# starlingonearth/MASt3R-SLAM-Quality-dualTSDF

Measured on AMD Instinct MI355X. Metric: SLAM frames/sec (infer+match+TSDF+GN) @512x384, higher is better.
Workload: dtype bf16

## Files before the change

include/mslam_hip.h:

```cpp
#ifndef MSLAM_HIP_H
#define MSLAM_HIP_H

#include <stddef.h>
#include <stdint.h>

#ifdef __cplusplus
extern "C" {
#endif

#define MSLAM_OK 0
#define MSLAM_EINVAL (-1)
#define MSLAM_EHIP (-2)
#define MSLAM_ENOMEM (-3)
#define MSLAM_ENODEV (-4)

const char* mslam_last_error(void);
int mslam_abi_version(void);
int mslam_device_check(void);


int mslam_iter_proj(const float* rays_img_with_grad, const float* pts_3d_norm,
                    const float* p_init, float* p_new, uint8_t* converged, int b, int h, int w,
                    int n, int max_iter, float lambda_init, float cost_thresh, void* stream);

int mslam_refine_matches(const uint16_t* D11, const uint16_t* D21, const int64_t* p1,
                         int64_t* p1_new, int b, int h, int w, int n, int fdim, int radius,
                         int dilation_max, void* stream);

int mslam_prep_iter_proj(const float* X11, const float* X21, const int64_t* idx_init,
                         float* rays_img_with_grad, float* pts_3d_norm, float* p_init, int b, int h,
                         int w, void* stream);

int mslam_match_occlusion(const float* X11, const float* X21, const float* p, int64_t* p1,
                          uint8_t* valid, int b, int h, int w, float dist_thresh, void* stream);

int mslam_pixel_to_lin(const int64_t* p1, int64_t* idx, int b, int n, int w, void* stream);

size_t mslam_gn_workspace_bytes(int num_poses, int num_edges, int num_points, int local_edges);

int mslam_gauss_newton_rays(float* Twc, const float* Xs, const float* Cs, const int64_t* ii,
                            const int64_t* jj, const int64_t* idx_ii2jj, const uint8_t* valid_match,
                            const float* Q, int num_poses, int num_points, int num_edges,
                            float sigma_ray, float sigma_dist, float C_thresh, float Q_thresh,
                            int max_iter, float delta_thresh, float* dx, void* workspace,
                            size_t workspace_bytes, void* stream);

int mslam_gauss_newton_calib(float* Twc, const float* Xs, const float* Cs, const float* K,
                             const int64_t* ii, const int64_t* jj, const int64_t* idx_ii2jj,
                             const uint8_t* valid_match, const float* Q, int num_poses, int num_points,
                             int num_edges, int height, int width, int pixel_border, float z_eps,
                             float sigma_pixel, float sigma_depth, float C_thresh, float Q_thresh,
                             int max_iter, float delta_thresh, float* dx, void* workspace,
                             size_t workspace_bytes, void* stream);

int mslam_gauss_newton_points(float* Twc, const float* Xs, const float* Cs, const int64_t* ii,
                              const int64_t* jj, const int64_t* idx_ii2jj, const uint8_t* valid_match,
                              const float* Q, int num_poses, int num_points, int num_edges,
                              float sigma_point, float C_thresh, float Q_thresh, int max_iter,
                              float delta_thresh, float* dx, void* workspace, size_t workspace_bytes,
// ... 265 lines not shown
                            uint8_t* out_count, void* stream);

#define MSLAM_IMAGE_METRICS_TILE_H 16
#define MSLAM_IMAGE_METRICS_TILE_W 32
size_t mslam_image_metrics_workspace_bytes(int n, int h, int w, int c);
int mslam_image_metrics(const float* a, const float* b, const uint8_t* mask, int n, int h, int w, int c,
                        const double* window, double* sums, int64_t* counts, float* ssim_map, void* workspace,
                        void* stream);

int mslam_mast3r_create(void** handle_out, const int* cfg9_host, void* const* weight_ptrs_host,
                        const long long* weight_numels_host, int n_weights, void* stream);
int mslam_mast3r_destroy(void* handle);
size_t mslam_mast3r_workspace_bytes(void* handle, int batch, int H, int W);

int mslam_mast3r_encode(void* handle, const float* img, int batch, int H, int W, float* feat_out,
                        void* workspace, size_t workspace_bytes, void* stream);

int mslam_mast3r_decode(void* handle, const float* feat1, const float* feat2, int batch, int H, int W,
                        float* X1, float* C1, float* D1, float* Q1, float* X2, float* C2, float* D2,
                        float* Q2, float* dec_last1, float* dec_last2, void* workspace,
                        size_t workspace_bytes, void* stream);

size_t mslam_track_workspace_bytes(int n_points);
int mslam_track_pose(int use_calib, float* T_rel, const float* Xf, const float* Xk, const int64_t* idx_f2k,
                     const float* Qk, const uint8_t* valid, int n_points, const float* K, int width,
                     int height, float sigma_a, float sigma_b, float huber, int pixel_border, float z_eps,
                     int first_iter, int max_iters, float rel_error, float delta_norm, void* status_out, void* workspace,
                     size_t workspace_bytes, void* stream);

size_t mslam_track_prepare_workspace_bytes(int n_points);
int mslam_track_prepare(const int64_t* idx_f2k, const uint8_t* valid_match, const float* Qff, const float* Qkf,
                        const float* Cf_sum, float inv_nf, const float* Ck_sum, float inv_nk, float C_conf, float Q_conf,
                        int n_points, const float* T_WCk, const float* T_WCf, float* Qk, float* Ck_avg,
                        uint8_t* valid_opt, uint8_t* valid_kf, float* T_rel, void* workspace, size_t workspace_bytes,
                        void* stream);
int mslam_track_verdict(const void* prepare_workspace, const void* status, int n_points, float* verdict6, void* stream);
int mslam_track_fuse(const float* T_WCk, const float* T_rel, const float* Xkf, const float* Ckf, const float* X_canon,
                     const float* C, int n_points, float* T_WCf, float* X_new, float* C_new, void* stream);

int mslam_gemm_bf16(const void* A, const void* W, const float* bias, const void* residual_f32, void* out,
                    int M, int N, int K, int act, int out_is_bf16, void* stream);
int mslam_gemm_tile_override(int M, int N, int K, int cfg);
int mslam_gemm_profile_begin(int M, int N, int K, int max_samples);
int mslam_gemm_profile_end(double* avg_us, double* min_us, int* samples);
int mslam_conv2d_nhwc_bf16(const void* in, const void* W, const float* bias, const void* residual_bf16,
                           void* out_bf16, int B, int H, int Wd, int Cin, int Cout, int ks, int stride,
// ... 64 lines not shown
```

mast3r-slam-quality-dualtsdf_amd/csrc/matching.hip:

```cpp
#include "common.h"

namespace mslam {

struct Bilin {
  float w11, w12, w21, w22;
  const float *r11, *r12, *r21, *r22;
};

__device__ __forceinline__ Bilin bilin_setup(const float* __restrict__ img, int w, float u, float v) {
  Bilin s;
  const int u11 = (int)floorf(u);
  const int v11 = (int)floorf(v);
  const float du = u - (float)u11;
  const float dv = v - (float)v11;
  const double dud = (double)du, dvd = (double)dv;
  const double omu = 1.0 - dud, omv = 1.0 - dvd;
  s.w11 = du * dv;
  s.w12 = (float)(omu * dvd);
  s.w21 = (float)(dud * omv);
  s.w22 = (float)(omu * omv);
  const float* base = img + ((size_t)v11 * w + u11) * 9;
  s.r22 = base;
  s.r21 = base + 9;
  s.r12 = base + (size_t)w * 9;
// ... 86 lines not shown
  converged[o] = conv;
}

typedef _Float16 h16;
typedef _Float16 h16x8 __attribute__((ext_vector_type(8)));

template <int FDIM>
__device__ __forceinline__ h16 half_dot_seq(const h16* __restrict__ a_regs, const h16* __restrict__ d11) {
  h16 score = (h16)0.0f;
  static_assert(FDIM % 8 == 0, "FDIM must be a multiple of 8");
#pragma unroll
  for (int c = 0; c < FDIM / 8; c++) {
    const h16x8 d = *reinterpret_cast<const h16x8*>(d11 + c * 8);
#pragma unroll
    for (int k = 0; k < 8; k++) {
      const h16 prod = a_regs[c * 8 + k] * d[k];
      score = score + prod;
    }
  }
  return score;
}

template <int FDIM>
__global__ __launch_bounds__(256) void refine_matches_kernel(
    const h16* __restrict__ D11, const h16* __restrict__ D21, const int64_t* __restrict__ p1,
    int64_t* __restrict__ p1_new, int h, int w, int n, int fdim_rt, int radius, int dilation_max) {
  const unsigned tile = xcd_remap(blockIdx.x, gridDim.x);
  const int i = tile * 256 + threadIdx.x;
  const int bi = blockIdx.y;
  if (i >= n) return;
  const int fdim = FDIM > 0 ? FDIM : fdim_rt;
  const h16* img = D11 + (size_t)bi * h * w * fdim;
  const size_t o = (size_t)bi * n + i;
  const h16* d21 = D21 + o * fdim;

  h16 a[FDIM > 0 ? FDIM : 1];
  if constexpr (FDIM > 0) {
#pragma unroll
    for (int c = 0; c < FDIM / 8; c++) {
      const h16x8 t = *reinterpret_cast<const h16x8*>(d21 + c * 8);
#pragma unroll
      for (int k = 0; k < 8; k++) a[c * 8 + k] = t[k];
    }
  }

  const longlong2 pp = *reinterpret_cast<const longlong2*>(p1 + o * 2);
  long long u0 = pp.x, v0 = pp.y;
  long long u_new = u0, v_new = v0;
  float max_score = 6.103515625e-05f;

  for (int d = dilation_max; d > 0; d--) {
    const int rd = radius * d;
    const int diam = 2 * rd + 1;
    for (int ii = 0; ii < diam; ii += d) {
      const long long u = u0 - rd + ii;
      const int ui = (int)u;
      if (ui < 0 || ui >= w) continue;
      for (int jj = 0; jj < diam; jj += d) {
        const long long v = v0 - rd + jj;
        const int vi = (int)v;
        if (vi < 0 || vi >= h) continue;
        const h16* d11 = img + ((unsigned)vi * (unsigned)w + (unsigned)ui) * (unsigned)fdim;
        h16 score;
        if constexpr (FDIM > 0) {
          score = half_dot_seq<FDIM>(a, d11);
        } else {
          score = (h16)0.0f;
          for (int k = 0; k < fdim; k++) {
            const h16 prod = d21[k] * d11[k];
            score = score + prod;
          }
        }
        const float sf = (float)score;
        if (sf > max_score) {
          max_score = sf;
          u_new = u;
          v_new = v;
        }
      }
    }
    u0 = u_new;
    v0 = v_new;
  }
  longlong2 out;
  out.x = u_new;
  out.y = v_new;
  *reinterpret_cast<longlong2*>(p1_new + o * 2) = out;
}

__device__ __forceinline__ int reflect_idx(int i, int n) {
  if (i < 0) return -i;
  if (i >= n) return 2 * n - 2 - i;
  return i;
}

__device__ __forceinline__ void normalize3(float x, float y, float z, float& ox, float& oy, float& oz) {
  const float nrm = fmaxf(sqrtf(fmaf(z, z, fmaf(y, y, x * x))), 1e-12f);
  ox = x / nrm;
  oy = y / nrm;
  oz = z / nrm;
}

constexpr int kPrepTile = 16;

__global__ __launch_bounds__(256) void prep_iter_proj_kernel(
    const float* __restrict__ X11, const float* __restrict__ X21, const int64_t* __restrict__ idx_init,
// ... 35 lines not shown
    gx = fmaf(-k3, a20, gx);
    gx = fmaf(k3, a22, gx);
    float gy = -k3 * a00;
    gy = fmaf(-k10, a01, gy);
    gy = fmaf(-k3, a02, gy);
    gy = fmaf(k3, a20, gy);
    gy = fmaf(k10, a21, gy);
    gy = fmaf(k3, a22, gy);
    out[c] = a11;
    out[3 + c] = gx;
    out[6 + c] = gy;
  }
  const float* q = X21 + o * 3;
  float a, b, c;
  normalize3(q[0], q[1], q[2], a, b, c);
  pts_out[o * 3 + 0] = a;
  pts_out[o * 3 + 1] = b;
  pts_out[o * 3 + 2] = c;
  const long long lin = idx_init ? idx_init[o] : (long long)pix;
  p_init[o * 2 + 0] = (float)(lin % w);
  p_init[o * 2 + 1] = (float)(lin / w);
}

__global__ __launch_bounds__(256) void match_occlusion_kernel(
    const float* __restrict__ X11, const float* __restrict__ X21, const float* __restrict__ p,
    int64_t* __restrict__ p1, uint8_t* __restrict__ valid, int h, int w, float dist_thresh) {
  const int n = h * w;
  const int i = blockIdx.x * 256 + threadIdx.x;
  const int bi = blockIdx.y;
  if (i >= n) return;
  const size_t o = (size_t)bi * n + i;
  const float2 pp = *reinterpret_cast<const float2*>(p + o * 2);
  const long long u = (long long)pp.x, v = (long long)pp.y;
  const float* a = X11 + ((size_t)bi * n + (size_t)v * w + (size_t)u) * 3;
  const float* q = X21 + o * 3;
  const float d0 = a[0] - q[0], d1 = a[1] - q[1], d2 = a[2] - q[2];
  const float dist = sqrtf(fmaf(d2, d2, fmaf(d1, d1, d0 * d0)));
  longlong2 out;
  out.x = u;
  out.y = v;
  *reinterpret_cast<longlong2*>(p1 + o * 2) = out;
  valid[o] = (valid[o] != 0) && (dist < dist_thresh);
}

__global__ __launch_bounds__(256) void pixel_to_lin_kernel(const int64_t* __restrict__ p1,
                                                           int64_t* __restrict__ idx, size_t total, int w) {
  const size_t i = (size_t)blockIdx.x * 256 + threadIdx.x;
  if (i >= total) return;
  const longlong2 pp = *reinterpret_cast<const longlong2*>(p1 + i * 2);
  idx[i] = pp.x + (long long)w * pp.y;
}

}

using namespace mslam;

extern "C" int mslam_iter_proj(const float* rays_img_with_grad, const float* pts_3d_norm,
                               const float* p_init, float* p_new, uint8_t* converged, int b, int h,
                               int w, int n, int max_iter, float lambda_init, float cost_thresh,
                               void* stream) {
  MSLAM_REQUIRE(b >= 0 && n >= 0 && max_iter >= 0, "iter_proj: negative size");
  if (b == 0 || n == 0) return MSLAM_OK;
  MSLAM_REQUIRE(rays_img_with_grad && pts_3d_norm && p_init && p_new && converged,
                "iter_proj: null pointer");
  MSLAM_REQUIRE(h >= 3 && w >= 3, "iter_proj: ray image must be at least 3x3 (got %dx%d)", h, w);
// ... 37 lines not shown
  MSLAM_REQUIRE(X11 && X21 && rays_img_with_grad && pts_3d_norm && p_init, "prep_iter_proj: null pointer");
  MSLAM_REQUIRE(h >= 2 && w >= 2, "prep_iter_proj: reflect padding needs h,w >= 2");
  MSLAM_REQUIRE(b <= 65535, "prep_iter_proj: batch %d exceeds grid limit", b);
  dim3 grid((w + kPrepTile - 1) / kPrepTile, (h + kPrepTile - 1) / kPrepTile, b);
  hipLaunchKernelGGL(prep_iter_proj_kernel, grid, dim3(256), 0, (hipStream_t)stream, X11, X21, idx_init,
                     rays_img_with_grad, pts_3d_norm, p_init, h, w);
  MSLAM_LAUNCH_CHECK("prep_iter_proj");
  return MSLAM_OK;
}

extern "C" int mslam_match_occlusion(const float* X11, const float* X21, const float* p, int64_t* p1,
                                     uint8_t* valid, int b, int h, int w, float dist_thresh,
                                     void* stream) {
  MSLAM_REQUIRE(b >= 0 && h >= 0 && w >= 0, "match_occlusion: negative size");
  if (b == 0 || h == 0 || w == 0) return MSLAM_OK;
  MSLAM_REQUIRE(X11 && X21 && p && p1 && valid, "match_occlusion: null pointer");
  dim3 grid((h * w + 255) / 256, b);
  hipLaunchKernelGGL(match_occlusion_kernel, grid, dim3(256), 0, (hipStream_t)stream, X11, X21, p, p1,
                     valid, h, w, dist_thresh);
  MSLAM_LAUNCH_CHECK("match_occlusion");
  return MSLAM_OK;
}

extern "C" int mslam_pixel_to_lin(const int64_t* p1, int64_t* idx, int b, int n, int w, void* stream) {
  MSLAM_REQUIRE(b >= 0 && n >= 0, "pixel_to_lin: negative size");
  const size_t total = (size_t)b * n;
  if (total == 0) return MSLAM_OK;
  MSLAM_REQUIRE(p1 && idx, "pixel_to_lin: null pointer");
  hipLaunchKernelGGL(pixel_to_lin_kernel, dim3((unsigned)((total + 255) / 256)), dim3(256), 0,
                     (hipStream_t)stream, p1, idx, total, w);
  MSLAM_LAUNCH_CHECK("pixel_to_lin");
  return MSLAM_OK;
}
```

mast3r-slam-quality-dualtsdf_amd/csrc/tracker.hip:

```cpp
#include "common.h"
#include "sim3.h"

namespace mslam {

constexpr int kTAcc = 36;

struct TrackState {
  int done;
  int iters;
  int chol_fail;
  float old_cost;
  float last_cost;
  float last_delta_norm;
  float pad0, pad1;
};

struct TrackParams {
  float inv_sigma_a, inv_sigma_b;
  float huber_k;
  const float* K;
  float border_lo, border_hi_u, border_hi_v, z_eps;
  int width;
};

__device__ __forceinline__ float huber_k(float r, float k) {
  const float a = fabsf(r);
  return a < k ? 1.0f : k / a;
}

template <unsigned NZ>
__device__ __forceinline__ void taccum_row(float (&acc)[kTAcc], const float (&x)[7], float w, float err) {
  const float we = w * err;
  int l = 0;
#pragma unroll
  for (int n = 0; n < 7; n++) {
    const float wx = w * x[n];
#pragma unroll
    for (int m = 0; m <= n; m++) {
      if (((NZ >> n) & 1u) && ((NZ >> m) & 1u)) acc[l] = fmaf(wx, x[m], acc[l]);
      l++;
    }
    if ((NZ >> n) & 1u) acc[28 + n] = fmaf(we, x[n], acc[28 + n]);
  }
  acc[35] = fmaf(we, err, acc[35]);
}

template <int CALIB>
__global__ __launch_bounds__(256) void track_accum_kernel(const TrackState* __restrict__ st,
                                                          const float* __restrict__ T,
                                                          const float* __restrict__ Xf, const float* __restrict__ Xk,
                                                          const int64_t* __restrict__ idx, const float* __restrict__ Qk,
                                                          const uint8_t* __restrict__ valid, int n, TrackParams P,
                                                          float* __restrict__ partial) {
  if (st->done) return;
  const Sim3f Tr = sim3_load(T);
  float R[9];
  quat_to_mat(Tr.q, R);
  float acc[kTAcc];
#pragma unroll
  for (int l = 0; l < kTAcc; l++) acc[l] = 0.0f;
  for (int k = blockIdx.x * 256 + threadIdx.x; k < n; k += gridDim.x * 256) {
    const long long j = idx[k];
    const float xf0 = Xf[j * 3], xf1 = Xf[j * 3 + 1], xf2 = Xf[j * 3 + 2];
    const float xk0 = Xk[(size_t)k * 3], xk1 = Xk[(size_t)k * 3 + 1], xk2 = Xk[(size_t)k * 3 + 2];
    const float p0 = Tr.s * (R[0] * xf0 + R[1] * xf1 + R[2] * xf2) + Tr.t[0];
    const float p1 = Tr.s * (R[3] * xf0 + R[4] * xf1 + R[5] * xf2) + Tr.t[1];
    const float p2 = Tr.s * (R[6] * xf0 + R[7] * xf1 + R[8] * xf2) + Tr.t[2];
    const float vq = valid[k] ? sqrtf(Qk[k]) : 0.0f;
    if constexpr (CALIB == 0) {
      const float nk = sqrtf(xk0 * xk0 + xk1 * xk1 + xk2 * xk2), nk_inv = 1.0f / nk;
      const float n2 = p0 * p0 + p1 * p1 + p2 * p2;
      const float np = sqrtf(n2), np_inv = 1.0f / np;
      const float r0 = p0 * np_inv, r1 = p1 * np_inv, r2 = p2 * np_inv;
      const float e0 = r0 - xk0 * nk_inv, e1 = r1 - xk1 * nk_inv, e2 = r2 - xk2 * nk_inv, e3 = np - nk;
      const float sa = P.inv_sigma_a * vq, sb = P.inv_sigma_b * vq;
      const float w0 = huber_k(sa * e0, P.huber_k) * sa * sa, w1 = huber_k(sa * e1, P.huber_k) * sa * sa;
      const float w2 = huber_k(sa * e2, P.huber_k) * sa * sa, w3 = huber_k(sb * e3, P.huber_k) * sb * sb;
      const float n3 = np_inv / n2;
// ... 21 lines not shown
      const float xz = p0 * zinv, yz = p1 * zinv;
      if (gate > 0.0f) {
        { const float x[7] = {Pfx * zinv, 0.0f, -Pfx * xz * zinv, -Pfx * xz * yz, Pfx * (1.0f + xz * xz), -Pfx * yz, 0.0f};
          taccum_row<0b0111101>(acc, x, w0, e0); }
        { const float x[7] = {0.0f, Pfy * zinv, -Pfy * yz * zinv, -Pfy * (1.0f + yz * yz), Pfy * xz * yz, Pfy * xz, 0.0f};
          taccum_row<0b0111110>(acc, x, w1, e1); }
        { const float x[7] = {0.0f, 0.0f, zinv, yz, -xz, 0.0f, 1.0f}; taccum_row<0b1011100>(acc, x, w2, e2); }
      }
    }
  }
  __shared__ float red[4][kTAcc];
  const int lane = threadIdx.x & 63, wid = threadIdx.x >> 6;
#pragma unroll
  for (int l = 0; l < kTAcc; l++) {
    const float s = wave_sum(acc[l]);
    if (lane == 0) red[wid][l] = s;
  }
  __syncthreads();
  if (threadIdx.x < kTAcc)
    partial[(size_t)blockIdx.x * kTAcc + threadIdx.x] =
        (red[0][threadIdx.x] + red[1][threadIdx.x]) + (red[2][threadIdx.x] + red[3][threadIdx.x]);
}

__global__ __launch_bounds__(64) void track_solve_kernel(TrackState* __restrict__ st, const float* __restrict__ partial,
                                                         int nblk, float* __restrict__ T, float rel_thresh,
                                                         float delta_thresh) {
  if (st->done) return;
  __shared__ double s[kTAcc];
  const int t = threadIdx.x;
  if (t < kTAcc) {
    double a = 0.0;
    for (int k = 0; k < nblk; k++) a += (double)partial[(size_t)k * kTAcc + t];
    s[t] = a;
  }
  __syncthreads();
  if (t != 0) return;
  double H[7][7], g[7];
  int l = 0;
  for (int n = 0; n < 7; n++)
    for (int m = 0; m <= n; m++) { H[n][m] = s[l]; H[m][n] = s[l]; l++; }
  for (int n = 0; n < 7; n++) g[n] = -s[28 + n];
  const float cost = (float)(0.5 * s[35]);
  double L[7][7];
  bool fail = false;
  for (int j = 0; j < 7 && !fail; j++) {
    double d = H[j][j];
    for (int k = 0; k < j; k++) d -= L[j][k] * L[j][k];
    if (!(d > 0.0)) { fail = true; break; }
    L[j][j] = sqrt(d);
    for (int i = j + 1; i < 7; i++) {
      double v = H[i][j];
      for (int k = 0; k < j; k++) v -= L[i][k] * L[j][k];
      L[i][j] = v / L[j][j];
    }
  }
  st->iters += 1;
  st->last_cost = cost;
  if (fail) { st->chol_fail = 1; st->done = 1; return; }
  double y[7], x[7];
  for (int i = 0; i < 7; i++) { double v = g[i]; for (int k = 0; k < i; k++) v -= L[i][k] * y[k]; y[i] = v / L[i][i]; }
  for (int i = 6; i >= 0; i--) { double v = y[i]; for (int k = i + 1; k < 7; k++) v -= L[k][i] * x[k]; x[i] = v / L[i][i]; }
  float tau[7];
  double nn = 0.0;
  for (int i = 0; i < 7; i++) { tau[i] = (float)x[i]; nn += (double)tau[i] * tau[i]; }
  sim3_store(T, sim3_unit(sim3_retr(tau, sim3_load(T))));
  const float delta_norm = (float)sqrt(nn);
  st->last_delta_norm = delta_norm;
  const float old = st->old_cost;
  const float rel_dec = fabsf((old - cost) / old);
  if (rel_dec < rel_thresh || delta_norm < delta_thresh) st->done = 1;
  st->old_cost = cost;
}

__global__ void track_init_kernel(TrackState* st) {
  st->done = 0; st->iters = 0; st->chol_fail = 0; st->old_cost = INFINITY; st->last_cost = 0.0f;
  st->last_delta_norm = 0.0f; st->pad0 = st->pad1 = 0.0f;
}

__device__ __host__ inline size_t prep_partials_bytes(int n) { return (((size_t)((n + 255) / 256) * 8) + 255) & ~(size_t)255; }

__global__ __launch_bounds__(256) void track_prep_kernel(
    const int64_t* __restrict__ idx, const uint8_t* __restrict__ vmatch, const float* __restrict__ Qff,
    const float* __restrict__ Qkf, const float* __restrict__ Cf_sum, float inv_nf, const float* __restrict__ Ck_sum,
    float inv_nk, float C_conf, float Q_conf, int n, const float* __restrict__ T_WCk, const float* __restrict__ T_WCf,
    float* __restrict__ Qk, float* __restrict__ Ck_avg, uint8_t* __restrict__ valid_opt, uint8_t* __restrict__ valid_kf,
    float* __restrict__ T_rel, int2* __restrict__ partial, uint8_t* __restrict__ hit) {
  const int k = blockIdx.x * 256 + threadIdx.x;
  if (k == 0) {
    const Sim3f Ti = sim3_unit(sim3_inv(sim3_load(T_WCk)));
    sim3_store(T_rel, sim3_unit(sim3_mul(Ti, sim3_load(T_WCf))));
  }
  bool opt = false, kf = false;
  if (k < n) {
    const long long j = idx[k];
    const bool vm = vmatch[k] != 0;
    const float q = sqrtf(Qff[j] * Qkf[k]);
    const float cf = Cf_sum[j] * inv_nf;
    const float ck = Ck_sum[k] * inv_nk;
    const bool vq = q > Q_conf;
// ... 47 lines not shown
}

__global__ __launch_bounds__(256) void track_fuse_kernel(const float* __restrict__ T_WCk, const float* __restrict__ T_rel,
                                                         const float* __restrict__ Xkf, const float* __restrict__ Ckf,
                                                         const float* __restrict__ Xc, const float* __restrict__ Cc, int n,
                                                         float* __restrict__ T_WCf, float* __restrict__ Xn,
                                                         float* __restrict__ Cn) {
  const int k = blockIdx.x * 256 + threadIdx.x;
  const Sim3f Tr = sim3_load(T_rel);
  if (k == 0) sim3_store(T_WCf, sim3_unit(sim3_mul(sim3_load(T_WCk), Tr)));
  if (k >= n) return;
  const float x[3] = {Xkf[(size_t)k * 3], Xkf[(size_t)k * 3 + 1], Xkf[(size_t)k * 3 + 2]};
  float y[3];
  sim3_act(Tr, x, y);
  const float c = Cc[k], cn = Ckf[k], den = c + cn;
#pragma unroll
  for (int d = 0; d < 3; d++) Xn[(size_t)k * 3 + d] = ((c * Xc[(size_t)k * 3 + d]) + (cn * y[d])) / den;
  Cn[k] = den;
}

}

using namespace mslam;

extern "C" size_t mslam_track_workspace_bytes(int n_points) {
  (void)n_points;
  return 256 + sizeof(float) * kTAcc * 1024;
}

extern "C" int mslam_track_pose(int use_calib, float* T_rel, const float* Xf, const float* Xk, const int64_t* idx_f2k,
                                const float* Qk, const uint8_t* valid, int n_points, const float* K, int width,
                                int height, float sigma_a, float sigma_b, float huber, int pixel_border, float z_eps,
                                int first_iter, int max_iters, float rel_error, float delta_norm, void* status_out,
                                void* workspace, size_t workspace_bytes, void* stream) {
  MSLAM_REQUIRE(n_points > 0 && max_iters >= 0 && first_iter >= 0, "track_pose: bad sizes");
  MSLAM_REQUIRE(T_rel && Xf && Xk && idx_f2k && Qk && valid && workspace, "track_pose: null pointer");
  MSLAM_REQUIRE(!use_calib || (K && width > 0 && height > 0), "track_pose: calib needs K, width, height");
  MSLAM_REQUIRE(workspace_bytes >= mslam_track_workspace_bytes(n_points), "track_pose: workspace too small");
  hipStream_t s = (hipStream_t)stream;
  TrackState* st = (TrackState*)workspace;
  float* partial = (float*)((char*)workspace + 256);
  int nblk = (n_points + 256 * 8 - 1) / (256 * 8);
  if (nblk > 1024) nblk = 1024;
  if (nblk < 1) nblk = 1;
  TrackParams P = {};
  P.inv_sigma_a = 1.0f / sigma_a; P.inv_sigma_b = 1.0f / sigma_b; P.huber_k = huber;
  P.width = width > 0 ? width : 1;
  if (use_calib) {
    P.K = K;
    P.border_lo = (float)pixel_border; P.border_hi_u = (float)(width - 1 - pixel_border);
    P.border_hi_v = (float)(height - 1 - pixel_border); P.z_eps = z_eps;
  }
  if (first_iter == 0) hipLaunchKernelGGL(track_init_kernel, dim3(1), dim3(1), 0, s, st);
  for (int it = first_iter; it < max_iters; it++) {
    if (use_calib)
      hipLaunchKernelGGL(track_accum_kernel<1>, dim3(nblk), dim3(256), 0, s, st, T_rel, Xf, Xk, idx_f2k, Qk, valid,
                         n_points, P, partial);
    else
      hipLaunchKernelGGL(track_accum_kernel<0>, dim3(nblk), dim3(256), 0, s, st, T_rel, Xf, Xk, idx_f2k, Qk, valid,
                         n_points, P, partial);
    hipLaunchKernelGGL(track_solve_kernel, dim3(1), dim3(64), 0, s, st, partial, nblk, T_rel, rel_error, delta_norm);
  }
  MSLAM_LAUNCH_CHECK("track_pose");
  if (status_out)
    return check_hip(hipMemcpyAsync(status_out, st, sizeof(TrackState), hipMemcpyDeviceToDevice, s), "track status");
  return MSLAM_OK;
}

extern "C" size_t mslam_track_prepare_workspace_bytes(int n_points) {
  return 256 + prep_partials_bytes(n_points) + (((size_t)n_points + 255) & ~(size_t)255);
}

extern "C" int mslam_track_prepare(const int64_t* idx_f2k, const uint8_t* valid_match, const float* Qff,
                                   const float* Qkf, const float* Cf_sum, float inv_nf, const float* Ck_sum,
                                   float inv_nk, float C_conf, float Q_conf, int n_points, const float* T_WCk,
                                   const float* T_WCf, float* Qk, float* Ck_avg, uint8_t* valid_opt, uint8_t* valid_kf,
                                   float* T_rel, void* workspace, size_t workspace_bytes, void* stream) {
  MSLAM_REQUIRE(n_points > 0, "track_prepare: bad sizes");
  MSLAM_REQUIRE(idx_f2k && valid_match && Qff && Qkf && Cf_sum && Ck_sum && T_WCk && T_WCf && Qk && Ck_avg && valid_opt &&
                    valid_kf && T_rel && workspace, "track_prepare: null pointer");
  MSLAM_REQUIRE(workspace_bytes >= mslam_track_prepare_workspace_bytes(n_points), "track_prepare: workspace too small");
  hipStream_t s = (hipStream_t)stream;
  MSLAM_REQUIRE(((uintptr_t)workspace & 15) == 0, "track_prepare: workspace must be 16-byte aligned");
  uint8_t* hit = (uint8_t*)workspace + 256 + prep_partials_bytes(n_points);
  int rc = check_hip(hipMemsetAsync(hit, 0, (size_t)n_points, s), "track_prepare: memset");
  if (rc) return rc;
  hipLaunchKernelGGL(track_prep_kernel, dim3((n_points + 255) / 256), dim3(256), 0, s, idx_f2k, valid_match, Qff, Qkf,
                     Cf_sum, inv_nf, Ck_sum, inv_nk, C_conf, Q_conf, n_points, T_WCk, T_WCf, Qk, Ck_avg, valid_opt,
// ... 26 lines not shown
```

mast3r-slam-quality-dualtsdf_amd/mast3r_slam/matching.py:

```python
import torch

import mast3r_slam_backends
import mslam_hip as _m
from mast3r_slam.config import config


def match(X11, X21, D11, D21, idx_1_to_2_init=None):
    idx_1_to_2, valid_match2 = match_iterative_proj(X11, X21, D11, D21, idx_1_to_2_init)
    return idx_1_to_2, valid_match2


def pixel_to_lin(p1, w):
    p1 = p1.contiguous()
    lead = p1.shape[:-1]
    n = 1
    for s in lead:
        n *= s
    idx = torch.empty(lead, dtype=torch.int64, device=p1.device)
    rc = _m.lib().mslam_pixel_to_lin(_m.ptr(p1), _m.ptr(idx), 1, n, int(w), _m.stream_ptr())
    _m.check(rc, "pixel_to_lin")
    return idx


def lin_to_pixel(idx_1_to_2, w):
# ... 12 lines not shown
    p_init = torch.empty((b, h * w, 2), dtype=torch.float32, device=dev)
    if idx_1_to_2_init is not None:
        idx_1_to_2_init = idx_1_to_2_init.contiguous()
        _m.require_dtype(idx_1_to_2_init, torch.int64, "idx_1_to_2_init")
    rc = _m.lib().mslam_prep_iter_proj(
        _m.ptr(X11), _m.ptr(X21), _m.ptr(idx_1_to_2_init), _m.ptr(rays), _m.ptr(pts), _m.ptr(p_init),
        b, h, w, _m.stream_ptr(),
    )
    _m.check(rc, "prep_for_iter_proj")
    return rays, pts, p_init


def match_iterative_proj(X11, X21, D11, D21, idx_1_to_2_init=None):
    cfg = config["matching"]
    b, h, w = X21.shape[:3]
    X11 = X11.contiguous()
    X21 = X21.contiguous()

    rays_with_grad_img, pts3d_norm, p_init = prep_for_iter_proj(X11, X21, idx_1_to_2_init)
    p1f, valid_proj2 = mast3r_slam_backends.iter_proj(
        rays_with_grad_img, pts3d_norm, p_init, cfg["max_iter"], cfg["lambda_init"], cfg["convergence_thresh"]
    )

    p1 = torch.empty((b, h * w, 2), dtype=torch.int64, device=X11.device)
    rc = _m.lib().mslam_match_occlusion(
        _m.ptr(X11), _m.ptr(X21), _m.ptr(p1f), _m.ptr(p1), _m.ptr(valid_proj2), b, h, w,
        float(cfg["dist_thresh"]), _m.stream_ptr(),
    )
    _m.check(rc, "match_occlusion")

    if cfg["radius"] > 0:
        (p1,) = mast3r_slam_backends.refine_matches(
            D11.half().contiguous(), D21.reshape(b, h * w, -1).half().contiguous(), p1,
            cfg["radius"], cfg["dilation_max"],
        )

    idx_1_to_2 = pixel_to_lin(p1, w)
    return idx_1_to_2, valid_proj2.unsqueeze(-1)
```

mast3r-slam-quality-dualtsdf_amd/mast3r_slam_backends.py:

```python
import torch

import mslam_hip as _m


def iter_proj(rays_img_with_grad, pts_3d_norm, p_init, max_iter, lambda_init, cost_thresh):
    _m.require_contiguous(rays_img_with_grad=rays_img_with_grad, pts_3d_norm=pts_3d_norm, p_init=p_init)
    for name, t in (("rays_img_with_grad", rays_img_with_grad), ("pts_3d_norm", pts_3d_norm), ("p_init", p_init)):
        _m.require_dtype(t, torch.float32, name)
    b, h, w, c = rays_img_with_grad.shape
    if c != 9:
        raise RuntimeError(f"rays_img_with_grad must have 9 channels, got {c}")
    n = p_init.shape[1]
    p_new = torch.empty((b, n, 2), dtype=p_init.dtype, device=p_init.device)
    converged = torch.empty((b, n), dtype=torch.bool, device=p_init.device)
    rc = _m.lib().mslam_iter_proj(
        _m.ptr(rays_img_with_grad), _m.ptr(pts_3d_norm), _m.ptr(p_init), _m.ptr(p_new), _m.ptr(converged),
        b, h, w, n, int(max_iter), float(lambda_init), float(cost_thresh), _m.stream_ptr(),
    )
    _m.check(rc, "iter_proj")
    return [p_new, converged]


def refine_matches(D11, D21, p1, radius, dilation_max):
    _m.require_contiguous(D11=D11, D21=D21, p1=p1)
    if D11.dtype != torch.float16 or D21.dtype != torch.float16:
        raise RuntimeError("refine_matches: D11/D21 must be float16 (the only dtype the SLAM path uses)")
    _m.require_dtype(p1, torch.int64, "p1")
    b, h, w, f = D11.shape
    n = p1.shape[1]
    p1_new = torch.empty((b, n, 2), dtype=p1.dtype, device=p1.device)
    rc = _m.lib().mslam_refine_matches(
        _m.ptr(D11), _m.ptr(D21), _m.ptr(p1), _m.ptr(p1_new), b, h, w, n, f, int(radius), int(dilation_max),
        _m.stream_ptr(),
    )
    _m.check(rc, "refine_matches")
    return [p1_new]


_ws_cache = {}


def _workspace(nbytes, device):
    key = (device.type, device.index)
    buf = _ws_cache.get(key)
    if buf is None or buf.numel() < nbytes:
        buf = torch.empty(int(nbytes * 1.25) + 1024, dtype=torch.uint8, device=device)
        _ws_cache[key] = buf
    return buf


def _gn_common_checks(Twc, Xs, Cs, ii, jj, idx_ii2jj, valid_match, Q):
    _m.require_contiguous(Twc=Twc, Xs=Xs, Cs=Cs, ii=ii, jj=jj, idx_ii2jj=idx_ii2jj, valid_match=valid_match, Q=Q)
    for name, t in (("Twc", Twc), ("Xs", Xs), ("Cs", Cs), ("Q", Q)):
        _m.require_dtype(t, torch.float32, name)
    for name, t in (("ii", ii), ("jj", jj), ("idx_ii2jj", idx_ii2jj)):
        _m.require_dtype(t, torch.int64, name)
    _m.require_dtype(valid_match, torch.bool, "valid_match")
    P, HW = Xs.shape[0], Xs.shape[1]
    E = ii.shape[0]
# ... 80 lines not shown
```

Baseline: 155.0.

## Fuse match occlusion/refine/lin kernels and merge tracker accumulate+solve via last-block ticket

Matching now runs occlusion check, descriptor refinement search and pixel-to-linear conversion in one kernel, which avoids writing and rereading the intermediate int64 p1 buffers and removes two launches. Tracking fuses the per-iteration accumulate and solve kernels into one: each block bumps an atomic ticket and the last block to arrive reduces the partials and runs the 7x7 Cholesky solve. This halves the tracker launches per iteration. In exchange it relies on correct memory fences and on resetting the counter. The old split path stays available behind a runtime switch.

```diff
diff --git a/include/mslam_hip.h b/include/mslam_hip.h
--- a/include/mslam_hip.h
+++ b/include/mslam_hip.h
@@ -35,6 +35,10 @@
                           uint8_t* valid, int b, int h, int w, float dist_thresh, void* stream);
 
 int mslam_pixel_to_lin(const int64_t* p1, int64_t* idx, int b, int n, int w, void* stream);
+
+int mslam_match_tail(const float* X11, const float* X21, const float* p, const uint16_t* D11, const uint16_t* D21,
+                     uint8_t* valid, int64_t* idx, int b, int h, int w, int fdim, int radius, int dilation_max,
+                     float dist_thresh, void* stream);
 
 size_t mslam_gn_workspace_bytes(int num_poses, int num_edges, int num_points, int local_edges);
 
@@ -346,6 +350,7 @@
                         size_t workspace_bytes, void* stream);
 
 size_t mslam_track_workspace_bytes(int n_points);
+int mslam_track_set_split(int on);
 int mslam_track_pose(int use_calib, float* T_rel, const float* Xf, const float* Xk, const int64_t* idx_f2k,
                      const float* Qk, const uint8_t* valid, int n_points, const float* K, int width,
                      int height, float sigma_a, float sigma_b, float huber, int pixel_border, float z_eps,
diff --git a/mast3r-slam-quality-dualtsdf_amd/csrc/matching.hip b/mast3r-slam-quality-dualtsdf_amd/csrc/matching.hip
--- a/mast3r-slam-quality-dualtsdf_amd/csrc/matching.hip
+++ b/mast3r-slam-quality-dualtsdf_amd/csrc/matching.hip
@@ -132,18 +132,9 @@
 }
 
 template <int FDIM>
-__global__ __launch_bounds__(256) void refine_matches_kernel(
-    const h16* __restrict__ D11, const h16* __restrict__ D21, const int64_t* __restrict__ p1,
-    int64_t* __restrict__ p1_new, int h, int w, int n, int fdim_rt, int radius, int dilation_max) {
-  const unsigned tile = xcd_remap(blockIdx.x, gridDim.x);
-  const int i = tile * 256 + threadIdx.x;
-  const int bi = blockIdx.y;
-  if (i >= n) return;
-  const int fdim = FDIM > 0 ? FDIM : fdim_rt;
-  const h16* img = D11 + (size_t)bi * h * w * fdim;
-  const size_t o = (size_t)bi * n + i;
-  const h16* d21 = D21 + o * fdim;
-
+__device__ __forceinline__ void refine_search(const h16* __restrict__ img, const h16* __restrict__ d21, long long u0,
+                                              long long v0, int h, int w, int fdim, int radius, int dilation_max,
+                                              long long& u_out, long long& v_out) {
   h16 a[FDIM > 0 ? FDIM : 1];
   if constexpr (FDIM > 0) {
 #pragma unroll
@@ -154,8 +145,6 @@
     }
   }
 
-  const longlong2 pp = *reinterpret_cast<const longlong2*>(p1 + o * 2);
-  long long u0 = pp.x, v0 = pp.y;
   long long u_new = u0, v_new = v0;
   float max_score = 6.103515625e-05f;
 
@@ -192,6 +181,24 @@
     u0 = u_new;
     v0 = v_new;
   }
+  u_out = u_new;
+  v_out = v_new;
+}
+
+template <int FDIM>
+__global__ __launch_bounds__(256) void refine_matches_kernel(
+    const h16* __restrict__ D11, const h16* __restrict__ D21, const int64_t* __restrict__ p1,
+    int64_t* __restrict__ p1_new, int h, int w, int n, int fdim_rt, int radius, int dilation_max) {
+  const unsigned tile = xcd_remap(blockIdx.x, gridDim.x);
+  const int i = tile * 256 + threadIdx.x;
+  const int bi = blockIdx.y;
+  if (i >= n) return;
+  const int fdim = FDIM > 0 ? FDIM : fdim_rt;
+  const h16* img = D11 + (size_t)bi * h * w * fdim;
+  const size_t o = (size_t)bi * n + i;
+  const longlong2 pp = *reinterpret_cast<const longlong2*>(p1 + o * 2);
+  long long u_new, v_new;
+  refine_search<FDIM>(img, D21 + o * fdim, pp.x, pp.y, h, w, fdim, radius, dilation_max, u_new, v_new);
   longlong2 out;
   out.x = u_new;
   out.y = v_new;
@@ -273,6 +280,20 @@
   p_init[o * 2 + 1] = (float)(lin / w);
 }
 
+__device__ __forceinline__ void occlusion_step(const float* __restrict__ X11, const float* __restrict__ X21,
+                                               const float* __restrict__ p, uint8_t* __restrict__ valid, int bi, int n,
+                                               int w, size_t o, float dist_thresh, long long& u_out, long long& v_out) {
+  const float2 pp = *reinterpret_cast<const float2*>(p + o * 2);
+  const long long u = (long long)pp.x, v = (long long)pp.y;
+  const float* a = X11 + ((size_t)bi * n + (size_t)v * w + (size_t)u) * 3;
+  const float* q = X21 + o * 3;
+  const float d0 = a[0] - q[0], d1 = a[1] - q[1], d2 = a[2] - q[2];
+  const float dist = sqrtf(fmaf(d2, d2, fmaf(d1, d1, d0 * d0)));
+  valid[o] = (valid[o] != 0) && (dist < dist_thresh);
+  u_out = u;
+  v_out = v;
+}
+
 __global__ __launch_bounds__(256) void match_occlusion_kernel(
     const float* __restrict__ X11, const float* __restrict__ X21, const float* __restrict__ p,
     int64_t* __restrict__ p1, uint8_t* __restrict__ valid, int h, int w, float dist_thresh) {
@@ -281,17 +302,31 @@
   const int bi = blockIdx.y;
   if (i >= n) return;
   const size_t o = (size_t)bi * n + i;
-  const float2 pp = *reinterpret_cast<const float2*>(p + o * 2);
-  const long long u = (long long)pp.x, v = (long long)pp.y;
-  const float* a = X11 + ((size_t)bi * n + (size_t)v * w + (size_t)u) * 3;
-  const float* q = X21 + o * 3;
-  const float d0 = a[0] - q[0], d1 = a[1] - q[1], d2 = a[2] - q[2];
-  const float dist = sqrtf(fmaf(d2, d2, fmaf(d1, d1, d0 * d0)));
+  long long u, v;
+  occlusion_step(X11, X21, p, valid, bi, n, w, o, dist_thresh, u, v);
   longlong2 out;
   out.x = u;
   out.y = v;
   *reinterpret_cast<longlong2*>(p1 + o * 2) = out;
-  valid[o] = (valid[o] != 0) && (dist < dist_thresh);
+}
+
+template <int FDIM>
+__global__ __launch_bounds__(256) void match_tail_kernel(
+    const float* __restrict__ X11, const float* __restrict__ X21, const float* __restrict__ p,
+    const h16* __restrict__ D11, const h16* __restrict__ D21, uint8_t* __restrict__ valid, int64_t* __restrict__ idx,
+    int h, int w, int fdim_rt, int radius, int dilation_max, float dist_thresh) {
+  const int n = h * w;
+  const unsigned tile = xcd_remap(blockIdx.x, gridDim.x);
+  const int i = tile * 256 + threadIdx.x;
+  const int bi = blockIdx.y;
+  if (i >= n) return;
+  const int fdim = FDIM > 0 ? FDIM : fdim_rt;
+  const size_t o = (size_t)bi * n + i;
+  long long u, v;
+  occlusion_step(X11, X21, p, valid, bi, n, w, o, dist_thresh, u, v);
+  long long u_new, v_new;
+  refine_search<FDIM>(D11 + (size_t)bi * n * fdim, D21 + o * fdim, u, v, h, w, fdim, radius, dilation_max, u_new, v_new);
+  idx[o] = u_new + (long long)w * v_new;
 }
 
 __global__ __launch_bounds__(256) void pixel_to_lin_kernel(const int64_t* __restrict__ p1,
@@ -375,6 +410,30 @@
   return MSLAM_OK;
 }
 
+extern "C" int mslam_match_tail(const float* X11, const float* X21, const float* p, const uint16_t* D11,
+                                const uint16_t* D21, uint8_t* valid, int64_t* idx, int b, int h, int w, int fdim,
+                                int radius, int dilation_max, float dist_thresh, void* stream) {
+  MSLAM_REQUIRE(b >= 0 && h >= 0 && w >= 0 && fdim >= 0, "match_tail: negative size");
+  if (b == 0 || h == 0 || w == 0) return MSLAM_OK;
+  MSLAM_REQUIRE(X11 && X21 && p && D11 && D21 && valid && idx, "match_tail: null pointer");
+  MSLAM_REQUIRE(b <= 65535, "match_tail: batch %d exceeds grid limit", b);
+  dim3 grid((h * w + 255) / 256, b);
+  const h16* d11 = reinterpret_cast<const h16*>(D11);
+  const h16* d21 = reinterpret_cast<const h16*>(D21);
+  if (fdim == 24) {
+    hipLaunchKernelGGL(match_tail_kernel<24>, grid, dim3(256), 0, (hipStream_t)stream, X11, X21, p, d11, d21, valid,
+                       idx, h, w, fdim, radius, dilation_max, dist_thresh);
+  } else if (fdim == 16) {
+    hipLaunchKernelGGL(match_tail_kernel<16>, grid, dim3(256), 0, (hipStream_t)stream, X11, X21, p, d11, d21, valid,
+                       idx, h, w, fdim, radius, dilation_max, dist_thresh);
+  } else {
+    hipLaunchKernelGGL(match_tail_kernel<0>, grid, dim3(256), 0, (hipStream_t)stream, X11, X21, p, d11, d21, valid,
+                       idx, h, w, fdim, radius, dilation_max, dist_thresh);
+  }
+  MSLAM_LAUNCH_CHECK("match_tail");
+  return MSLAM_OK;
+}
+
 extern "C" int mslam_pixel_to_lin(const int64_t* p1, int64_t* idx, int b, int n, int w, void* stream) {
   MSLAM_REQUIRE(b >= 0 && n >= 0, "pixel_to_lin: negative size");
   const size_t total = (size_t)b * n;
diff --git a/mast3r-slam-quality-dualtsdf_amd/csrc/tracker.hip b/mast3r-slam-quality-dualtsdf_amd/csrc/tracker.hip
--- a/mast3r-slam-quality-dualtsdf_amd/csrc/tracker.hip
+++ b/mast3r-slam-quality-dualtsdf_amd/csrc/tracker.hip
@@ -1,3 +1,5 @@
+#include <atomic>
+
 #include "common.h"
 #include "sim3.h"
 
@@ -46,14 +48,10 @@
 }
 
 template <int CALIB>
-__global__ __launch_bounds__(256) void track_accum_kernel(const TrackState* __restrict__ st,
-                                                          const float* __restrict__ T,
-                                                          const float* __restrict__ Xf, const float* __restrict__ Xk,
-                                                          const int64_t* __restrict__ idx, const float* __restrict__ Qk,
-                                                          const uint8_t* __restrict__ valid, int n, TrackParams P,
-                                                          float* __restrict__ partial) {
-  if (st->done) return;
-  const Sim3f Tr = sim3_load(T);
+__device__ __forceinline__ void track_accum_block(const Sim3f& Tr, const float* __restrict__ Xf,
+                                                  const float* __restrict__ Xk, const int64_t* __restrict__ idx,
+                                                  const float* __restrict__ Qk, const uint8_t* __restrict__ valid, int n,
+                                                  const TrackParams& P, float* partial) {
   float R[9];
   quat_to_mat(Tr.q, R);
   float acc[kTAcc];
@@ -121,6 +119,76 @@
         (red[0][threadIdx.x] + red[1][threadIdx.x]) + (red[2][threadIdx.x] + red[3][threadIdx.x]);
 }
 
+template <int CALIB>
+__global__ __launch_bounds__(256) void track_accum_kernel(const TrackState* __restrict__ st,
+                                                          const float* __restrict__ T,
+                                                          const float* __restrict__ Xf, const float* __restrict__ Xk,
+                                                          const int64_t* __restrict__ idx, const float* __restrict__ Qk,
+                                                          const uint8_t* __restrict__ valid, int n, TrackParams P,
+                                                          float* __restrict__ partial) {
+  if (st->done) return;
+  track_accum_block<CALIB>(sim3_load(T), Xf, Xk, idx, Qk, valid, n, P, partial);
+}
+
+__device__ __forceinline__ void track_solve_step(TrackState* st, const double* s, float* T, float rel_thresh,
+                                                 float delta_thresh) {
+  double H[7][7], g[7];
+  int l = 0;
+#pragma unroll
+  for (int n = 0; n < 7; n++)
+#pragma unroll
+    for (int m = 0; m <= n; m++) { H[n][m] = s[l]; H[m][n] = s[l]; l++; }
+#pragma unroll
+  for (int n = 0; n < 7; n++) g[n] = -s[28 + n];
+  const float cost = (float)(0.5 * s[35]);
+  double L[7][7];
+  bool fail = false;
+#pragma unroll
+  for (int j = 0; j < 7 && !fail; j++) {
+    double d = H[j][j];
+#pragma unroll
+    for (int k = 0; k < j; k++) d -= L[j][k] * L[j][k];
+    if (!(d > 0.0)) { fail = true; break; }
+    L[j][j] = sqrt(d);
+#pragma unroll
+    for (int i = j + 1; i < 7; i++) {
+      double v = H[i][j];
+#pragma unroll
+      for (int k = 0; k < j; k++) v -= L[i][k] * L[j][k];
+      L[i][j] = v / L[j][j];
+    }
+  }
+  st->iters += 1;
+  st->last_cost = cost;
+  if (fail) { st->chol_fail = 1; st->done = 1; return; }
+  double y[7], x[7];
+#pragma unroll
+  for (int i = 0; i < 7; i++) {
+    double v = g[i];
+#pragma unroll
+    for (int k = 0; k < i; k++) v -= L[i][k] * y[k];
+    y[i] = v / L[i][i];
+  }
+#pragma unroll
+  for (int i = 6; i >= 0; i--) {
+    double v = y[i];
+#pragma unroll
+    for (int k = i + 1; k < 7; k++) v -= L[k][i] * x[k];
+    x[i] = v / L[i][i];
+  }
+  float tau[7];
+  double nn = 0.0;
+#pragma unroll
+  for (int i = 0; i < 7; i++) { tau[i] = (float)x[i]; nn += (double)tau[i] * tau[i]; }
+  sim3_store(T, sim3_unit(sim3_retr(tau, sim3_load(T))));
+  const float delta_norm = (float)sqrt(nn);
+  st->last_delta_norm = delta_norm;
+  const float old = st->old_cost;
+  const float rel_dec = fabsf((old - cost) / old);
+  if (rel_dec < rel_thresh || delta_norm < delta_thresh) st->done = 1;
+  st->old_cost = cost;
+}
+
 __global__ __launch_bounds__(64) void track_solve_kernel(TrackState* __restrict__ st, const float* __restrict__ partial,
                                                          int nblk, float* __restrict__ T, float rel_thresh,
                                                          float delta_thresh) {
@@ -134,46 +202,68 @@
   }
   __syncthreads();
   if (t != 0) return;
-  double H[7][7], g[7];
-  int l = 0;
-  for (int n = 0; n < 7; n++)
-    for (int m = 0; m <= n; m++) { H[n][m] = s[l]; H[m][n] = s[l]; l++; }
-  for (int n = 0; n < 7; n++) g[n] = -s[28 + n];
-  const float cost = (float)(0.5 * s[35]);
-  double L[7][7];
-  bool fail = false;
-  for (int j = 0; j < 7 && !fail; j++) {
-    double d = H[j][j];
-    for (int k = 0; k < j; k++) d -= L[j][k] * L[j][k];
-    if (!(d > 0.0)) { fail = true; break; }
-    L[j][j] = sqrt(d);
-    for (int i = j + 1; i < 7; i++) {
-      double v = H[i][j];
-      for (int k = 0; k < j; k++) v -= L[i][k] * L[j][k];
-      L[i][j] = v / L[j][j];
-    }
-  }
-  st->iters += 1;
-  st->last_cost = cost;
-  if (fail) { st->chol_fail = 1; st->done = 1; return; }
-  double y[7], x[7];
-  for (int i = 0; i < 7; i++) { double v = g[i]; for (int k = 0; k < i; k++) v -= L[i][k] * y[k]; y[i] = v / L[i][i]; }
-  for (int i = 6; i >= 0; i--) { double v = y[i]; for (int k = i + 1; k < 7; k++) v -= L[k][i] * x[k]; x[i] = v / L[i][i]; }
-  float tau[7];
-  double nn = 0.0;
-  for (int i = 0; i < 7; i++) { tau[i] = (float)x[i]; nn += (double)tau[i] * tau[i]; }
-  sim3_store(T, sim3_unit(sim3_retr(tau, sim3_load(T))));
-  const float delta_norm = (float)sqrt(nn);
-  st->last_delta_norm = delta_norm;
-  const float old = st->old_cost;
-  const float rel_dec = fabsf((old - cost) / old);
-  if (rel_dec < rel_thresh || delta_norm < delta_thresh) st->done = 1;
-  st->old_cost = cost;
+  track_solve_step(st, s, T, rel_thresh, delta_thresh);
+}
+
+constexpr int kTicketOffset = 64;
+constexpr int kStageBlocks = 128;
+
+__device__ __forceinline__ void track_status_store(int* status_out, const TrackState* st) {
+  const int* src = reinterpret_cast<const int*>(st);
+#pragma unroll
+  for (int i = 0; i < (int)(sizeof(TrackState) / sizeof(int)); i++) status_out[i] = src[i];
+}
+
+template <int CALIB>
+__global__ __launch_bounds__(256) void track_iter_kernel(TrackState* st, float* T, const float* __restrict__ Xf,
+                                                         const float* __restrict__ Xk, const int64_t* __restrict__ idx,
+                                                         const float* __restrict__ Qk, const uint8_t* __restrict__ valid,
+                                                         int n, TrackParams P, float* partial, unsigned* counter,
+                                                         float rel_thresh, float delta_thresh, int* status_out) {
+  if (st->done) {
+    if (status_out && blockIdx.x == 0 && threadIdx.x == 0) track_status_store(status_out, st);
+    return;
+  }
+  track_accum_block<CALIB>(sim3_load(T), Xf, Xk, idx, Qk, valid, n, P, partial);
+  __shared__ float stage[kStageBlocks * kTAcc];
+  __shared__ double s[kTAcc];
+  __shared__ int is_last;
+  const int t = threadIdx.x;
+  if (t < kTAcc) {
+    __threadfence();
+    asm volatile("s_waitcnt vmcnt(0)" ::: "memory");
+  }
+  __syncthreads();
+  if (t == 0) {
+    const unsigned ticket = __hip_atomic_fetch_add(counter, 1u, __ATOMIC_ACQ_REL, __HIP_MEMORY_SCOPE_AGENT);
+    is_last = ticket == gridDim.x - 1;
+  }
+  __syncthreads();
+  if (!is_last) return;
+  const int nblk = gridDim.x;
+  double a = 0.0;
+  for (int k0 = 0; k0 < nblk; k0 += kStageBlocks) {
+    const int kn = min(kStageBlocks, nblk - k0);
+    const float* src = partial + (size_t)k0 * kTAcc;
+    for (int e = t; e < kn * kTAcc; e += 256)
+      stage[e] = __hip_atomic_load(src + e, __ATOMIC_RELAXED, __HIP_MEMORY_SCOPE_AGENT);
+    __syncthreads();
+    if (t < kTAcc)
+      for (int k = 0; k < kn; k++) a += (double)stage[k * kTAcc + t];
+    __syncthreads();
+  }
+  if (t < kTAcc) s[t] = a;
+  __syncthreads();
+  if (t != 0) return;
+  track_solve_step(st, s, T, rel_thresh, delta_thresh);
+  if (status_out) track_status_store(status_out, st);
+  __hip_atomic_store(counter, 0u, __ATOMIC_RELAXED, __HIP_MEMORY_SCOPE_AGENT);
 }
 
 __global__ void track_init_kernel(TrackState* st) {
   st->done = 0; st->iters = 0; st->chol_fail = 0; st->old_cost = INFINITY; st->last_cost = 0.0f;
   st->last_delta_norm = 0.0f; st->pad0 = st->pad1 = 0.0f;
+  *reinterpret_cast<unsigned*>(reinterpret_cast<char*>(st) + kTicketOffset) = 0u;
 }
 
 __device__ __host__ inline size_t prep_partials_bytes(int n) { return (((size_t)((n + 255) / 256) * 8) + 255) & ~(size_t)255; }
@@ -267,6 +357,8 @@
 }
 
 using namespace mslam;
+
+static std::atomic<int> g_track_split{0};
 
 extern "C" size_t mslam_track_workspace_bytes(int n_points) {
   (void)n_points;
@@ -297,18 +389,38 @@
     P.border_hi_v = (float)(height - 1 - pixel_border); P.z_eps = z_eps;
   }
   if (first_iter == 0) hipLaunchKernelGGL(track_init_kernel, dim3(1), dim3(1), 0, s, st);
-  for (int it = first_iter; it < max_iters; it++) {
-    if (use_calib)
-      hipLaunchKernelGGL(track_accum_kernel<1>, dim3(nblk), dim3(256), 0, s, st, T_rel, Xf, Xk, idx_f2k, Qk, valid,
-                         n_points, P, partial);
-    else
-      hipLaunchKernelGGL(track_accum_kernel<0>, dim3(nblk), dim3(256), 0, s, st, T_rel, Xf, Xk, idx_f2k, Qk, valid,
-                         n_points, P, partial);
-    hipLaunchKernelGGL(track_solve_kernel, dim3(1), dim3(64), 0, s, st, partial, nblk, T_rel, rel_error, delta_norm);
-  }
-  MSLAM_LAUNCH_CHECK("track_pose");
+  const bool split = g_track_split.load(std::memory_order_relaxed) != 0;
+  if (!split) {
+    unsigned* counter = (unsigned*)((char*)workspace + kTicketOffset);
+    for (int it = first_iter; it < max_iters; it++) {
+      if (use_calib)
+        hipLaunchKernelGGL(track_iter_kernel<1>, dim3(nblk), dim3(256), 0, s, st, T_rel, Xf, Xk, idx_f2k, Qk, valid,
+                           n_points, P, partial, counter, rel_error, delta_norm, (int*)status_out);
+      else
+        hipLaunchKernelGGL(track_iter_kernel<0>, dim3(nblk), dim3(256), 0, s, st, T_rel, Xf, Xk, idx_f2k, Qk, valid,
+                           n_points, P, partial, counter, rel_error, delta_norm, (int*)status_out);
+    }
+    MSLAM_LAUNCH_CHECK("track_pose");
+    if (first_iter < max_iters || !status_out) return MSLAM_OK;
+  } else {
+    for (int it = first_iter; it < max_iters; it++) {
+      if (use_calib)
+        hipLaunchKernelGGL(track_accum_kernel<1>, dim3(nblk), dim3(256), 0, s, st, T_rel, Xf, Xk, idx_f2k, Qk, valid,
+                           n_points, P, partial);
+      else
+        hipLaunchKernelGGL(track_accum_kernel<0>, dim3(nblk), dim3(256), 0, s, st, T_rel, Xf, Xk, idx_f2k, Qk, valid,
+                           n_points, P, partial);
+      hipLaunchKernelGGL(track_solve_kernel, dim3(1), dim3(64), 0, s, st, partial, nblk, T_rel, rel_error, delta_norm);
+    }
+    MSLAM_LAUNCH_CHECK("track_pose");
+  }
   if (status_out)
     return check_hip(hipMemcpyAsync(status_out, st, sizeof(TrackState), hipMemcpyDeviceToDevice, s), "track status");
+  return MSLAM_OK;
+}
+
+extern "C" int mslam_track_set_split(int on) {
+  g_track_split.store(on != 0 ? 1 : 0, std::memory_order_relaxed);
   return MSLAM_OK;
 }
 
diff --git a/mast3r-slam-quality-dualtsdf_amd/mast3r_slam/matching.py b/mast3r-slam-quality-dualtsdf_amd/mast3r_slam/matching.py
--- a/mast3r-slam-quality-dualtsdf_amd/mast3r_slam/matching.py
+++ b/mast3r-slam-quality-dualtsdf_amd/mast3r_slam/matching.py
@@ -58,18 +58,18 @@
         rays_with_grad_img, pts3d_norm, p_init, cfg["max_iter"], cfg["lambda_init"], cfg["convergence_thresh"]
     )
 
+    if cfg["radius"] > 0:
+        (idx_1_to_2,) = mast3r_slam_backends.match_tail(
+            X11, X21, p1f, D11.half().contiguous(), D21.reshape(b, h * w, -1).half().contiguous(), valid_proj2,
+            cfg["radius"], cfg["dilation_max"], cfg["dist_thresh"],
+        )
+        return idx_1_to_2, valid_proj2.unsqueeze(-1)
+
     p1 = torch.empty((b, h * w, 2), dtype=torch.int64, device=X11.device)
     rc = _m.lib().mslam_match_occlusion(
         _m.ptr(X11), _m.ptr(X21), _m.ptr(p1f), _m.ptr(p1), _m.ptr(valid_proj2), b, h, w,
         float(cfg["dist_thresh"]), _m.stream_ptr(),
     )
     _m.check(rc, "match_occlusion")
-
-    if cfg["radius"] > 0:
-        (p1,) = mast3r_slam_backends.refine_matches(
-            D11.half().contiguous(), D21.reshape(b, h * w, -1).half().contiguous(), p1,
-            cfg["radius"], cfg["dilation_max"],
-        )
-
     idx_1_to_2 = pixel_to_lin(p1, w)
     return idx_1_to_2, valid_proj2.unsqueeze(-1)
diff --git a/mast3r-slam-quality-dualtsdf_amd/mast3r_slam_backends.py b/mast3r-slam-quality-dualtsdf_amd/mast3r_slam_backends.py
--- a/mast3r-slam-quality-dualtsdf_amd/mast3r_slam_backends.py
+++ b/mast3r-slam-quality-dualtsdf_amd/mast3r_slam_backends.py
@@ -35,6 +35,23 @@
     )
     _m.check(rc, "refine_matches")
     return [p1_new]
+
+
+def match_tail(X11, X21, p, D11, D21, valid, radius, dilation_max, dist_thresh):
+    _m.require_contiguous(X11=X11, X21=X21, p=p, D11=D11, D21=D21, valid=valid)
+    for name, t in (("X11", X11), ("X21", X21), ("p", p)):
+        _m.require_dtype(t, torch.float32, name)
+    if D11.dtype != torch.float16 or D21.dtype != torch.float16:
+        raise RuntimeError("match_tail: D11/D21 must be float16 (the only dtype the SLAM path uses)")
+    _m.require_dtype(valid, torch.bool, "valid")
+    b, h, w, f = D11.shape
+    idx = torch.empty((b, h * w), dtype=torch.int64, device=p.device)
+    rc = _m.lib().mslam_match_tail(
+        _m.ptr(X11), _m.ptr(X21), _m.ptr(p), _m.ptr(D11), _m.ptr(D21), _m.ptr(valid), _m.ptr(idx), b, h, w, f,
+        int(radius), int(dilation_max), float(dist_thresh), _m.stream_ptr(),
+    )
+    _m.check(rc, "match_tail")
+    return [idx]
 
 
 _ws_cache = {}
```

New measurement: 148.1. 0.955x the previous value.
